# novara754/arctic-renderer

Measured on AMD Instinct MI355X. Metric: Mshaded-pixels/sec at 4K Sponza, 1 dir + 64 point lights; HBM GB/s vs roofline, higher is better.
Workload: dtype f32

## Files before the change

### arctic-renderer_amd/binding.py

```python
import ctypes as C
import os
import re

from .scene import CCreateInfo, CScene, CSettings

HERE = os.path.dirname(os.path.abspath(__file__))
LIB_PATH = os.environ.get("ARCTIC_HIP_LIBRARY") or os.path.join(HERE, "csrc", "libarctic_hip.so")
HEADER_PATH = os.path.join(os.path.dirname(HERE), "include", "arctic_hip.h")

OPTIONS = {"keep_float_output": 1, "count_light_evals": 2, "culling": 3, "debug": 4, "antialias": 5, "hdr16": 6, "ray_refit": 7, "shadow_cache": 9, "visbuffer": 10, "item_table_floor": 11, "light_path": 12, "markers": 13, "shadow_sharded": 14, "frames_in_flight": 15, "tiles_per_wave": 16, "tile_trace": 17, "raster_owner": 18, "tile_order": 19, "order_tail": 20, "sampler": 21, "texture_tiling": 22, "cluster_cull": 23, "small_triangles": 24, "env_lighting": 25, "point_shadow_size": 26, "texture_mips": 27}
TRACE_ANY, TRACE_BRUTE = 1, 2
ERRORS = {-1: "ARCTIC_E_INVALID", -2: "ARCTIC_E_DEVICE", -3: "ARCTIC_E_NO_DEVICE", -4: "ARCTIC_E_STATE", -5: "ARCTIC_E_CAPACITY"}

_vp, _u32, _u64, _i32, _i64 = C.c_void_p, C.c_uint32, C.c_uint64, C.c_int32, C.c_int64
_scene, _settings = C.POINTER(CScene), C.POINTER(CSettings)

SIGNATURES = {
    "arctic_create": (_vp, [C.POINTER(CCreateInfo), C.c_char_p, _u64]),
    "arctic_destroy": (None, [_vp]),
    "arctic_last_error": (C.c_char_p, [_vp]),
    "arctic_resize": (_i32, [_vp, _u32, _u32]),
    "arctic_flush": (_i32, [_vp]),
    "arctic_set_stream": (_i32, [_vp, _vp]),
    "arctic_use_own_stream": (_i32, [_vp]),
    "arctic_create_material": (_i32, [_vp, _vp, _u32, _u32, _vp, _u32, _u32, _vp, _u32, _u32]),
    "arctic_create_mesh": (_i32, [_vp, _vp, _u64, _vp, _u64, _u64]),
    "arctic_set_mesh_skin": (_i32, [_vp, _u64, _vp, _u64, _u32]),
    "arctic_set_mesh_pose": (_i32, [_vp, _u64, _vp, _u32]),
    "arctic_set_mesh_morph_targets": (_i32, [_vp, _u64, _vp, _u64, _u32]),
    "arctic_set_mesh_morph_weights": (_i32, [_vp, _u64, _vp, _u32]),
    "arctic_check_morph_targets": (_i32, [_vp, _u64, _u32]),
    "arctic_morph_vertices": (_i32, [_vp, _vp, _u64, _u32, _vp, _vp]),
    "arctic_read_mesh_vertices": (_i32, [_vp, _u64, _vp, _u64]),
    "arctic_check_mesh_skin": (_i32, [_vp, _u64, _u32]),
    "arctic_skin_vertices": (_i32, [_vp, _vp, _u64, _vp, _u32, _vp]),
    "arctic_set_material_extras": (_i32, [_vp, _u64, _vp, _vp, _u32, _u32, _vp, _u32, _u32]),
    "arctic_check_material_params": (_i32, [_vp]),
    "arctic_update_lights": (_i32, [_vp, _vp, _u64]),
    "arctic_update_spot_lights": (_i32, [_vp, _vp, _u64]),
    "arctic_spot_light_constants": (_i32, [_vp, _u64, _vp]),
    "arctic_update_point_shadow_lights": (_i32, [_vp, _vp, _u64]),
    "arctic_point_shadow_matrices": (_i32, [_vp, _vp]),
    "arctic_pass_point_shadows": (_i32, [_vp, _scene]),
    "arctic_read_point_shadow": (_i32, [_vp, _u32, _vp]),
    "arctic_write_point_shadow": (_i32, [_vp, _u32, _vp]),
    "arctic_create_hdri": (_i32, [_vp, _vp, _u32, _u32]),
    "arctic_render_frame": (_i32, [_vp, _scene, _settings, _vp]),
    "arctic_render_frame_device": (_i32, [_vp, _scene, _settings, _vp]),
    "arctic_pass_shadow_map": (_i32, [_vp, _scene]),
    "arctic_pass_gbuffer": (_i32, [_vp, _scene]),
    "arctic_pass_shade": (_i32, [_vp, _scene, _settings, _vp]),
    "arctic_post_process": (_i32, [_vp, _vp, _u32, _u32, _settings, _vp, _vp]),
    "arctic_antialias_device": (_i32, [_vp, _vp, _vp, _u32, _u32]),
# ... 76 lines not shown
```

### arctic-renderer_amd/csrc/common.h

```cpp
#pragma once
#include <hip/hip_runtime.h>
#include <stdint.h>
#include <stddef.h>
#include <algorithm>

namespace arctic {

constexpr int TILE = 8;
constexpr int TILE_PIXELS = 64;
constexpr uint32_t NO_MATERIAL = 0xFFFFFFFFu;
constexpr uint32_t MAX_TARGET = 16384;

struct GBuffer {
    float4 *a;
    float *b;
    float4 *c, *d, *e;
};
__host__ __device__ inline void gbuffer_pack(const float *v , uint32_t mat, float4 &A, float *B3, float4 &C, float4 &D, float4 &E) {
    A = make_float4(v[0], v[1], v[14], v[15]);
    B3[0] = v[16]; B3[1] = v[17]; B3[2] = __builtin_bit_cast(float, mat);
    C = make_float4(v[11], v[12], v[13], v[2]);
    D = make_float4(v[3], v[4], v[5], v[6]);
    E = make_float4(v[7], v[8], v[9], v[10]);
}
// ... 152 lines not shown
    const TexDesc *tex;
    const float2 *shadow_bounds;
    const float *shadow_map;
    uint8_t *out_rgba8;
    uint32_t shadow_size;
    uint32_t bounds_pitch;
    uint32_t width;
    uint32_t rows;
    uint32_t row0_in_tile;
    int32_t culling;
    int32_t hdr16;
    int32_t tm_method;
    float ambient;
    float inv_gamma;
    float exposure;
    uint32_t pad_c0;
    float *out_ldr;
    float *out_hdr;
    float eye[3];
    uint32_t n_lights;
    const float4 *light_pairs;
    const float4 *lights;
    float sun_dir[3];
    uint32_t n_spots;
    float sun_color[3];
    uint32_t n_cubes;
    const float *srgb_lut;
    union {
        unsigned long long *stats;
        const float4 *spots;
    };
// ... 7 lines not shown
    };
    uint32_t n_jobs;
    uint32_t cube_size;
    union {
        const unsigned long long *vis;
        const float *lod;
    };
    const SetupRec *recs; const RasterRec *rrecs; const uint32_t *rec_of; const ObjectRec *objs; const XVert *xv;
    const float4 *env;
    uint32_t env_w, env_h;
    float sky_fwd[3], sky_right[3], sky_up[3];
    float ndc_sx, ndc_sy;
    int32_t band_tiles, shard_index, shard_count, tile_y0;
    int32_t compact_tables;
};
static_assert(offsetof(ShadeParams, tex) == 64 && offsetof(ShadeParams, ambient) == 128 && offsetof(ShadeParams, sun_dir) == 192 &&
              offsetof(ShadeParams, srgb_lut) == 224, "ShadeParams: the blocks k_material loads in one batch each");
struct ShadeLaunch {
    hipStream_t stream;
    uint32_t loop;
    uint32_t from_vis;
    uint32_t stats;
    uint32_t tiles_per_wave;
    uint32_t env;
    uint32_t spot;
    uint32_t mip;
    uint32_t cube;
    uint32_t pbr;
};

// ... 21 lines not shown
    w = std::max(8u, std::min(W, 512u) >> (k - 1));
    h = std::max(4u, std::min(H, 256u) >> (k - 1));
}
inline uint32_t env_mip_count(uint32_t W, uint32_t H) { uint32_t n = 1; while (W > 1 || H > 1) { W = std::max(1u, W >> 1); H = std::max(1u, H >> 1); ++n; } return n; }
struct EnvBuild {
    const float4 *env; uint32_t W, H;
    float4 *levels;
    float2 *lut;
    float4 *mips;
    double *sh_rows;
    EnvTables *tables;
};
size_t env_levels_bytes(uint32_t W, uint32_t H);
size_t env_mips_bytes(uint32_t W, uint32_t H);
hipError_t launch_env_build(const EnvBuild &b, hipStream_t s);
constexpr uint32_t N_SHADE_STATS = 9;
constexpr uint32_t DEFAULT_TILES_PER_WAVE = 2;
constexpr uint32_t ORDER_NONE = 0xFFFFFFFFu;
__host__ __device__ inline uint32_t order_slot(uint32_t list, uint32_t i, uint32_t group) { return ((i / group) * 8u + list) * group + i % group; }
__host__ __device__ inline uint32_t order_slots(uint32_t tiles_x, uint32_t tiles_y, uint32_t group) {
    const uint32_t longest = ((tiles_x + 3) / 4) * ((tiles_y + 7) / 8);
    return 8u * ((longest + group - 1) / group * group);
}
constexpr uint32_t SMALL_FRAME_TILES = 48000;
inline uint32_t shadow_bounds_pitch(uint32_t S) { return S >= 4 && S <= 4900 ? (S + 3) / 4 : 0; }

hipError_t launch_vertex(const ObjectRec *objs, const uint32_t *block_obj, const uint32_t *block_first,
                         uint32_t n_blocks, const GeomParams &gp, XVert *xv, int clip_only, uint32_t *counters ,
                         unsigned long long *clear, unsigned long long clear_value, size_t clear_count ,
                         uint32_t *zero, size_t zero_count ,
                         const float *block_bounds , hipStream_t s);
// ... 57 lines not shown
```

### arctic-renderer_amd/csrc/renderer.cpp

```cpp
#include <algorithm>
#include <cstdarg>
#include <cstdio>
#include <dlfcn.h>

#include <cstdlib>
#include <cstring>
#include <cmath>
#include <limits>
#include <string>
#include <vector>

#include "../../include/arctic_hip.h"
#include "../../include/arctic_dist.h"
#include "common.h"
#include "ray_query.h"

using namespace arctic;

namespace {

struct Markers {
    int (*push)(const char *) = nullptr;
    int (*pop)() = nullptr;
    bool tried = false, on = false;
// ... 215 lines not shown
    uint32_t n_spots = 0;
    DevBuf d_cubes;
    uint32_t n_cubes = 0, cube_size = 1024;
    std::vector<ArcticPointShadowLight> cube_lights;
    std::vector<uint8_t> cube_key;
    uint32_t *h_cube_counts = nullptr, *dh_cube_counts = nullptr;
    uint32_t cube_count_faces = 0;
    DevBuf d_vis_set[3], d_p0, d_p1, d_p2, d_p3, d_p4, d_rgba8, d_ldr, d_hdr, d_counter;
    bool have_gbuffer = false, have_output = false, have_vis = false;
    int antialias = 0;
    DevBuf d_aa;
    bool output_filtered = false;
    bool aa_active() const { return antialias == 1 && rows() == height; }
    const void *rgba8_output() const { return output_filtered ? d_aa.p : d_rgba8.p; }
    int light_path = 0;
    bool visbuffer = true;
    PassTables tables[4];
    struct GeoSet {
        DevBuf d_xverts, d_recs, d_rrecs, d_clip_list, d_rec_of, d_items;
        DevBuf d_left;
        DevBuf d_bin_count, d_bin_slots;
        uint32_t item_cap = 0;
        uint32_t bins_x = 0, bins_y = 0;
        uint32_t n_tblocks = 0, n_vblocks = 0; bool cull_counted = false;
    } geo[4];
    DevBuf d_geo_counters, d_stage;
    hipStream_t shadow_stream = nullptr;
    hipEvent_t ev_fork = nullptr, ev_shadow = nullptr;
    hipEvent_t ev_skin = nullptr;
    uint64_t skin_seq = 0, skin_seen_shadow = 0, skin_seen_prepass[2] = {0, 0};
// ... 489 lines not shown
    std::memset(&sp, 0, sizeof sp);
    sp.g = r->gbuffer();
    const ArcticRenderer::GeoSet &G = r->geo[r->fwd()];
    sp.compact_tables = (G.d_recs.cap < (1ull << 32) && G.d_rrecs.cap < (1ull << 32) && G.d_xverts.cap < (1ull << 32) && G.d_rec_of.cap < (1ull << 32) &&
                         r->tables[r->fwd()].d.cap < (1ull << 32) && !(r->debug & 64)) ? 1 : 0;
    sp.vis = r->d_vis().as<unsigned long long>();
    if (!from_vis && r->mips_active()) sp.lod = r->d_lod.as<float>();
    sp.recs = G.d_recs.as<SetupRec>(); sp.rrecs = G.d_rrecs.as<RasterRec>(); sp.rec_of = G.d_rec_of.as<uint32_t>();
    sp.objs = r->tables[r->fwd()].objs; sp.xv = G.d_xverts.as<XVert>();
    sp.tex = r->d_tex.as<TexDesc>();
    sp.n_materials = (uint32_t)(r->tex.size() / 3);
    sp.srgb_lut = r->d_lut.as<float>();
    sp.shadow_map = r->shadow_size ? r->d_shadow().as<float>() : nullptr;
    sp.shadow_size = r->shadow_size;
    sp.lights = r->d_lights.as<float4>(); sp.light_pairs = r->d_light_pairs.as<float4>();
    sp.n_lights = r->n_lights;
    std::memcpy(sp.eye, sc->camera.eye, 12);
    dir_from_rot(sc->sun.rotation, sp.sun_dir);
    std::memcpy(sp.sun_color, sc->sun.color, 12);
    sp.ambient = sc->ambient;
    sp.tm_method = st->tm_method;
    sp.inv_gamma = 1.0f / st->gamma;
    sp.exposure = st->exposure;
    sp.width = r->width; sp.rows = r->rows(); sp.row0_in_tile = r->row0_in_tile;
    sp.tiles_x = r->tiles_x; sp.tiles_y = r->tiles_y;
    sp.out_rgba8 = static_cast<uint8_t *>(d_out && !r->aa_active() ? d_out : r->d_rgba8.p);
    size_t out_px = (size_t)r->rows() * r->width;
    if (r->keep_float) {
        HIPCHECK(r, r->d_ldr.ensure(out_px * 12));
        HIPCHECK(r, r->d_hdr.ensure(out_px * 12));
        sp.out_ldr = r->d_ldr.as<float>(); sp.out_hdr = r->d_hdr.as<float>();
// ... 60 lines not shown
        if (f.ptr && (f.ptr == static_cast<const void *>(sp.out_rgba8) || f.ptr == aa_out)) { HIPCHECK(r, hipStreamWaitEvent(r->stream, f.done, 0)); f.ptr = nullptr; }
    if (r->count_evals) {
        sp.stats = r->d_counter.as<unsigned long long>();
        HIPCHECK(r, hipMemsetAsync(r->d_counter.p, 0, 8 * N_SHADE_STATS, r->stream));
    }
    HIPCHECK(r, shade_once(r, sp, from_vis, r->count_evals != 0));
    if (aa) {
        Range aa_zone("Anti-aliasing Pass");
        HIPCHECK(r, launch_antialias(r->d_rgba8.p, aa_out, r->width, r->rows(), r->stream));
    }
    if (r->count_evals) {
        unsigned long long n[N_SHADE_STATS] = {};
        HIPCHECK(r, hipMemcpyAsync(n, r->d_counter.p, 8 * N_SHADE_STATS, hipMemcpyDeviceToHost, r->stream));
        HIPCHECK(r, hipStreamSynchronize(r->stream));
        r->stats[5] = n[0]; r->stats[6] = n[1]; r->stats[7] = n[2];
        r->light_stats[0] = n[3]; r->light_stats[1] = n[4];
        for (int i = 0; i < 4; ++i) r->edge_stats[i] = n[5 + i];
    }
    r->have_output = (d_out == nullptr);
    r->output_filtered = aa && d_out == nullptr;
    return ARCTIC_OK;
}

std::vector<uint8_t> shadow_inputs(const ArcticRenderer *r, const ArcticScene *sc) {
    std::vector<uint8_t> k;
    if (!r->shadow_size) return k;
    auto put = [&](const void *p, size_t n) { const uint8_t *b = static_cast<const uint8_t *>(p); k.insert(k.end(), b, b + n); };
    const uint64_t head[3] = {r->shadow_size, (uint64_t)r->meshes.size(), sc->n_objects};
    put(head, sizeof head);
    put(sc->sun.position, sizeof sc->sun.position);
    put(sc->sun.rotation, sizeof sc->sun.rotation);
// ... 556 lines not shown
    return ARCTIC_OK;
}

int arctic_read_mesh_vertices(ArcticRenderer *r, uint64_t mesh, ArcticVertex *out, uint64_t n_vertices) {
    if (!r) return ARCTIC_E_INVALID;
    if (mesh >= r->meshes.size()) return r->fail(ARCTIC_E_INVALID, "read_mesh_vertices: mesh %llu does not exist", (unsigned long long)mesh);
    const Mesh &m = r->meshes[mesh];
    if (!out || n_vertices != m.n_vertices) return r->fail(ARCTIC_E_INVALID, "read_mesh_vertices: room for %llu vertices, the mesh has %u", (unsigned long long)n_vertices, m.n_vertices);
    int rc = select_device(r);
    if (rc) return rc;
    HIPCHECK(r, hipStreamSynchronize(r->stream));
    HIPCHECK(r, hipMemcpy(out, m.vertices_in_use(), n_vertices * sizeof(ArcticVertex), hipMemcpyDeviceToHost));
    return ARCTIC_OK;
}

int arctic_update_lights(ArcticRenderer *r, const ArcticPointLight *lights, uint64_t n) {
    if (!r) return ARCTIC_E_INVALID;
    if (n && !lights) return r->fail(ARCTIC_E_INVALID, "update_lights: null");
    int rc = select_device(r);
    if (rc) return rc;
    uint32_t k = (uint32_t)std::min<uint64_t>(n, r->max_lights);
    HIPCHECK(r, hipStreamSynchronize(r->stream));
    if (k) HIPCHECK(r, hipMemcpy(r->d_lights.p, lights, (size_t)k * sizeof(ArcticPointLight), hipMemcpyHostToDevice));
    {
        const uint32_t n_pairs = (k + 1) / 2;
        std::vector<float> pairs((size_t)std::max(1u, n_pairs) * 12, 0.0f);
        for (uint32_t i = 0; i < 2 * n_pairs; ++i) {
            float *dst = pairs.data() + (size_t)(i / 2) * 12 + (i & 1);
            if (i < k) { dst[0] = lights[i].position[0]; dst[2] = lights[i].position[1]; dst[4] = lights[i].position[2];
                         dst[6] = lights[i].color[0]; dst[8] = lights[i].color[1]; dst[10] = lights[i].color[2]; }
            else { dst[0] = 0.0f; dst[2] = 1.0e6f; dst[4] = 0.0f; dst[6] = dst[8] = dst[10] = 0.0f; }
        }
        HIPCHECK(r, r->d_light_pairs.ensure(pairs.size() * 4));
        HIPCHECK(r, hipMemcpy(r->d_light_pairs.p, pairs.data(), pairs.size() * 4, hipMemcpyHostToDevice));
    }
    r->n_lights = k;
    return ARCTIC_OK;
}

int arctic_spot_light_constants(const ArcticSpotLight *lights, uint64_t n, float *out) {
    if (n && (!lights || !out)) return ARCTIC_E_INVALID;
    const float PI_F = (float)M_PI;
    for (uint64_t i = 0; i < n; ++i) {
        const ArcticSpotLight &l = lights[i];
        const float *f = l.position;
        for (int k = 0; k < 12; ++k) if (!std::isfinite(f[k])) return ARCTIC_E_INVALID;
        const double dx = l.direction[0], dy = l.direction[1], dz = l.direction[2];
        if (dx == 0.0 && dy == 0.0 && dz == 0.0) return ARCTIC_E_INVALID;
        if (!(l.inner_cone_angle >= 0.0f && l.inner_cone_angle <= l.outer_cone_angle && l.outer_cone_angle > 0.0f && l.outer_cone_angle <= PI_F &&
              l.range >= 0.0f)) return ARCTIC_E_INVALID;
// ... 636 lines not shown
            for (hipStream_t ps : r->prepass_stream) if (ps) HIPCHECK(r, hipStreamSynchronize(ps));
            if (r->own_stream_is_prepass()) HIPCHECK(r, hipStreamSynchronize(r->own_stream));
            if (r->cur >= (int)value) { r->cur = 0; r->have_vis = r->have_gbuffer = r->have_order = false; }
            r->released_valid[0] = r->released_valid[1] = r->released_valid[2] = false;
        }
        r->frames_in_flight = (int)value;
        break;
    case ARCTIC_OPT_MARKERS:
        g_markers.enable(value != 0);
        if (value && !g_markers.available()) return r->fail(ARCTIC_E_STATE, "set_option: libroctx64.so could not be loaded");
        break;
    case ARCTIC_OPT_LIGHT_PATH:
        if (value < 0 || value > 2) return r->fail(ARCTIC_E_INVALID, "set_option: light path must be 0..2");
        r->light_path = (int)value;
        break;
    case ARCTIC_OPT_ITEM_TABLE_FLOOR:
        if (value < 64 || value > 0x7FFFFFF0ll) return r->fail(ARCTIC_E_INVALID, "set_option: item table floor out of range");
        r->item_cap_floor = (uint32_t)value; r->geo[0].item_cap = r->geo[1].item_cap = r->geo[2].item_cap = r->geo[3].item_cap = 0;
        break;
    case ARCTIC_OPT_TILES_PER_WAVE:
        if (value < 0 || value > 64) return r->fail(ARCTIC_E_INVALID, "set_option: tiles per wave must be 0 (default) .. 64");
        r->tiles_per_wave = (uint32_t)value;
        break;
    case ARCTIC_OPT_TILE_TRACE: r->tile_trace = value != 0; break;
    case ARCTIC_OPT_TEXTURE_TILING: r->texture_tiling = value < 0 ? -1 : (value != 0); break;
    case ARCTIC_OPT_TEXTURE_MIPS:
        if (value < 0 || value > 1) return r->fail(ARCTIC_E_INVALID, "ARCTIC_OPT_TEXTURE_MIPS: 0 or 1");
        if ((int)value != r->texture_mips) r->lod_valid = false;
        r->texture_mips = (int)value;
        break;
// ... 531 lines not shown
```

### arctic-renderer_amd/csrc/shade.hip

```cpp
#include "common.h"
#include "edges.h"
#include "shadow_coords.h"
#include "texture_lod.h"

namespace arctic {

namespace {

typedef const ShadeParams __attribute__((address_space(4))) &SP;
typedef const ShadeParams __attribute__((address_space(4))) *KernArgs;

struct ArgsA { const float4 *ga; const float *gb; uint32_t tiles_x, tiles_y, T, stride; int32_t debug; uint32_t n_materials; };
__device__ __forceinline__ ArgsA args_a(KernArgs a) {
    ArgsA r = {a->g.a, a->g.b, a->tiles_x, a->tiles_y, a->tiles_per_wave, a->group_stride, a->debug, a->n_materials};
    asm volatile("" : "+s"(r.ga), "+s"(r.gb), "+s"(r.tiles_x), "+s"(r.tiles_y), "+s"(r.T), "+s"(r.stride), "+s"(r.debug), "+s"(r.n_materials));
    return r;
}
typedef const uint32_t __attribute__((address_space(4))) *OrderList;
struct OrderArgs { OrderList order; uint32_t n_jobs; };
__device__ __forceinline__ ArgsA args_a_first(KernArgs a, const float *&srgb_lut, const unsigned long long *&vis, OrderArgs &O) {
    ArgsA r = {a->g.a, a->g.b, a->tiles_x, a->tiles_y, a->tiles_per_wave, a->group_stride, a->debug, a->n_materials};
    srgb_lut = a->srgb_lut; vis = a->vis;
    const uint32_t *order = a->tile_order; O.n_jobs = a->n_jobs;
    asm volatile("" : "+s"(r.ga), "+s"(r.gb), "+s"(r.tiles_x), "+s"(r.tiles_y), "+s"(r.T), "+s"(r.stride), "+s"(r.debug), "+s"(r.n_materials), "+s"(srgb_lut), "+s"(vis),
// ... 22 lines not shown
struct ArgsC { float ambient; StoreArgs st; const float4 *gc, *gd, *ge; };
__device__ __forceinline__ ArgsC args_c(KernArgs a, const ArgsA &A, const ArgsB &B) {
    ArgsC r = {a->ambient, {B.hdr16, A.debug, B.tm, a->exposure, a->inv_gamma, a->out_ldr, a->out_hdr}, a->g.c, a->g.d, a->g.e};
    asm volatile("" : "+s"(r.ambient), "+s"(r.st.exposure), "+s"(r.st.inv_gamma), "+s"(r.st.out_ldr), "+s"(r.st.out_hdr), "+s"(r.gc), "+s"(r.gd), "+s"(r.ge));
    return r;
}
struct EpiArgs { StoreArgs st; uint8_t *out; uint32_t width, row0_in_tile; float ambient; };
__device__ __forceinline__ EpiArgs epi_args(KernArgs a) {
    EpiArgs r = {{a->hdr16, a->debug, a->tm_method, a->exposure, a->inv_gamma, a->out_ldr, a->out_hdr}, a->out_rgba8, a->width, a->row0_in_tile, a->ambient};
    asm volatile("" : "+s"(r.st.hdr16), "+s"(r.st.debug), "+s"(r.st.tm), "+s"(r.st.exposure), "+s"(r.st.inv_gamma), "+s"(r.st.out_ldr), "+s"(r.st.out_hdr), "+s"(r.out),
                 "+s"(r.width), "+s"(r.row0_in_tile), "+s"(r.ambient));
    return r;
}
__device__ __forceinline__ ShadowArgs shadow_args(SP sp) { ShadowArgs r = {sp.shadow_map, sp.shadow_bounds, sp.shadow_size, sp.bounds_pitch}; return r; }
__device__ __forceinline__ StoreArgs store_args(SP sp) { StoreArgs r = {sp.hdr16, sp.debug, sp.tm_method, sp.exposure, sp.inv_gamma, sp.out_ldr, sp.out_hdr}; return r; }
struct LightArgs { float eye[3]; uint32_t n_lights; const float4 *pairs, *lights; };
__device__ __forceinline__ LightArgs light_args(SP sp) {
    LightArgs r = {{sp.eye[0], sp.eye[1], sp.eye[2]}, sp.n_lights, sp.light_pairs, sp.lights};
    asm volatile("" : "+s"(r.eye[0]), "+s"(r.eye[1]), "+s"(r.eye[2]), "+s"(r.n_lights), "+s"(r.pairs), "+s"(r.lights));
    return r;
}
struct SunArgs { float dir[3], color[3]; };
__device__ __forceinline__ SunArgs sun_args(SP sp) {
    SunArgs r = {{sp.sun_dir[0], sp.sun_dir[1], sp.sun_dir[2]}, {sp.sun_color[0], sp.sun_color[1], sp.sun_color[2]}};
    asm volatile("" : "+s"(r.dir[0]), "+s"(r.dir[1]), "+s"(r.dir[2]), "+s"(r.color[0]), "+s"(r.color[1]), "+s"(r.color[2]));
    return r;
}

struct f3 { float x, y, z; };
__device__ __forceinline__ f3 mk(float x, float y, float z) { f3 r; r.x = x; r.y = y; r.z = z; return r; }
__device__ __forceinline__ f3 operator+(f3 a, f3 b) { return mk(a.x + b.x, a.y + b.y, a.z + b.z); }
__device__ __forceinline__ f3 operator-(f3 a, f3 b) { return mk(a.x - b.x, a.y - b.y, a.z - b.z); }
__device__ __forceinline__ f3 operator*(f3 a, f3 b) { return mk(a.x * b.x, a.y * b.y, a.z * b.z); }
__device__ __forceinline__ f3 operator*(f3 a, float s) { return mk(a.x * s, a.y * s, a.z * s); }
// ... 365 lines not shown
    k.q21 = (v2){p.q2, p.q1}; k.q0_ = (v2){p.q0, 0.0f};
    return k;
}
typedef float f4v __attribute__((ext_vector_type(4)));
__device__ __forceinline__ void load_light_pair(const char *p , f4v &A, f4v &B, f4v &C) {
    asm volatile("s_load_dwordx4 %0, %3, 0x0\n\ts_load_dwordx4 %1, %3, 0x10\n\ts_load_dwordx4 %2, %3, 0x20" : "=&s"(A), "=&s"(B), "=&s"(C) : "s"(p));
}
__device__ __forceinline__ void wait_and_sub(v2 lx, v2 ly, v2 lz, v2 w_xy, v2 wz, v2 &dx, v2 &dy, v2 &dz) {
    asm volatile("s_waitcnt lgkmcnt(0)\n\t"
                 "v_pk_add_f32 %0, %3, %6 op_sel:[0,0] op_sel_hi:[1,0] neg_lo:[0,1] neg_hi:[0,1]\n\t"
                 "v_pk_add_f32 %1, %4, %6 op_sel:[0,1] op_sel_hi:[1,1] neg_lo:[0,1] neg_hi:[0,1]\n\t"
                 "v_pk_add_f32 %2, %5, %7 op_sel:[0,0] op_sel_hi:[1,0] neg_lo:[0,1] neg_hi:[0,1]"
                 : "=&v"(dx), "=&v"(dy), "=&v"(dz) : "s"(lx), "s"(ly), "s"(lz), "v"(w_xy), "v"(wz));
}

__device__ __forceinline__ v2 accumulate_pair(const PackedPix &k, v2 dx, v2 dy, v2 dz, v2 cr, v2 cg, v2 cb, Sums2 &S) {
    const v2 d2 = pk_fma(dz, dz, pk_fma(dy, dy, dx * dx));
    v2 ndx;
    const v2 inv = rsq2_and_mul_b0(d2, dx, k.n_xy, ndx);
    const v2 nd = pk_fma_b1<0>(dz, k.nz_wox, pk_fma_b1<1>(dy, k.n_xy, ndx));
    const v2 ndwi = pk_mul_sat(nd, inv);
    const v2 hx = pk_fma_b2<1>(dx, inv, k.nz_wox), hy = pk_fma_b2<0>(dy, inv, k.wo_yz), hz = pk_fma_b2<1>(dz, inv, k.wo_yz);
    const v2 hh = pk_fma(hz, hz, pk_fma(hy, hy, hx * hx));
    v2 q;
    const v2 rh = rsq2_and_fma_b01(hh, ndwi, k.q21, q);
    const v2 m = pk_fma(hh * rh, (v2){-0.5f, -0.5f}, (v2){1.0f, 1.0f});
    const v2 ex = pk_fnma_b2<0>(hx, rh, k.n_xy), ey = pk_fnma_b2<1>(hy, rh, k.n_xy), ez = pk_fnma_b2<0>(hz, rh, k.nz_wox);
    const v2 e2 = pk_fma(ez, ez, pk_fma(ey, ey, ex * ex));
    const v2 dd = pk_fma_b2<1>(e2, pk_fma_b12<1, 0>(e2, k.oma2_c4, k.oma2_c4), k.wz_a2);
    const v2 den = (dd * dd) * pk_fma_b2<0>(q, ndwi, k.q0_);
    const v2 sc = ndwi * (inv * inv);
    v2 m2;
    const v2 rden = rcp2_and_mul(den, m, m, m2);
    const v2 p5 = m2 * m2 * m;
    const v2 s2 = (sc * ndwi) * rden;
    const v2 s1 = pk_fma(-sc, p5, sc), s3 = s2 * p5;
    pk_fma_s(cr, s1, S.a[0]); pk_fma_s(cg, s1, S.a[1]); pk_fma_s(cb, s1, S.a[2]);
    pk_fma_s(cr, s2, S.b[0]); pk_fma_s(cg, s2, S.b[1]); pk_fma_s(cb, s2, S.b[2]);
    pk_fma_s(cr, s3, S.c[0]); pk_fma_s(cg, s3, S.c[1]); pk_fma_s(cb, s3, S.c[2]);
    return nd;
}

__device__ __forceinline__ float rrt_odt(float c) {
    float a = fm(c, c + 0.0245786f, -0.000090537f);
    float b = fm(c, fm(0.983729f, c, 0.4329510f), 0.238081f);
    return a * rcp(b);
}
__device__ __forceinline__ v2 pk_fma_sat(v2 k , v2 a, v2 c) { v2 r; asm("v_pk_fma_f32 %0, %1, %2, %3 clamp" : "=v"(r) : "s"(k), "v"(a), "v"(c)); return r; }
__device__ __forceinline__ float fma_sat(float k , float a, float c) { float r; asm("v_fma_f32 %0, %1, %2, %3 clamp" : "=v"(r) : "s"(k), "v"(a), "v"(c)); return r; }
__device__ __forceinline__ f3 tonemap(f3 c, int tm, float exposure) {
    f3 t;
    if (tm == 1) {
        const float LOG2E = 1.4426950408889634f;
        const f3 x = mk(c.x * exposure, c.y * exposure, c.z * exposure);
// ... 178 lines not shown
        C[0] = __builtin_fmaf(cr, s3, C[0]); C[1] = __builtin_fmaf(cg, s3, C[1]); C[2] = __builtin_fmaf(cb, s3, C[2]);
    }
}
template <int LOOP, bool STATS, bool SPOT = false, bool CUBE = false, bool PBR = false>
__device__ __forceinline__ f3 lit_radiance(SP sp, uint32_t lane, float nr, float ng, float nb, float rough, float metal, f3 base,
                                           const float4 &gc, const float4 &gd, const float4 &ge, float nscale = 1.0f ) {
    const f3 n = PBR ? get_normal_scaled(nr, ng, nb, gc, gd, ge, nscale) : get_normal(nr, ng, nb, gc, gd, ge);
    const f3 world = mk(gc.x, gc.y, gc.z);
    const LightArgs la = light_args(sp);
    const f3 wo = normalize(mk(la.eye[0], la.eye[1], la.eye[2]) - world);
    asm volatile("" : "+v"(metal));
    LoopPix px;
    TailPix tp;
    make_pix(n, wo, world, base, metal, rough, px, tp);
    unsigned long long contributing = 0ull, wave_zero = 0ull;
    f3 Lo;
    if (LOOP == 1) {
        Sums S;
        {
            const SunArgs sun = sun_args(sp);
            const f3 d = mk(-sun.dir[0], -sun.dir[1], -sun.dir[2]);
            float s1, s2, s3;
            light_scalars<false>(px, d, dot(n, d), s1, s2, s3);
            for (int k = 0; k < 3; ++k) { S.a[k] = sun.color[k] * s1; S.b[k] = sun.color[k] * s2; S.c[k] = sun.color[k] * s3; }
        }
        for (uint32_t i = 0; i < la.n_lights; ++i) {
            typedef const f4v __attribute__((address_space(4))) *const_f4;
            const f4v lp = ((const_f4)la.lights)[2 * i], lc = ((const_f4)la.lights)[2 * i + 1];
            const f3 dl = mk(lp.x, lp.y, lp.z) - world;
            const float ndl = dot(n, dl);
// ... 2 lines not shown
            float s1, s2, s3;
            light_scalars<true>(px, dl, ndl, s1, s2, s3);
            S.a[0] = __builtin_fmaf(lc.x, s1, S.a[0]); S.a[1] = __builtin_fmaf(lc.y, s1, S.a[1]); S.a[2] = __builtin_fmaf(lc.z, s1, S.a[2]);
            S.b[0] = __builtin_fmaf(lc.x, s2, S.b[0]); S.b[1] = __builtin_fmaf(lc.y, s2, S.b[1]); S.b[2] = __builtin_fmaf(lc.z, s2, S.b[2]);
            S.c[0] = __builtin_fmaf(lc.x, s3, S.c[0]); S.c[1] = __builtin_fmaf(lc.y, s3, S.c[1]); S.c[2] = __builtin_fmaf(lc.z, s3, S.c[2]);
        }
        if (SPOT) spot_sums(sp, px, S.a, S.b, S.c);
        if (CUBE) cube_sums(sp, px, S.a, S.b, S.c);
        Lo = resolve_sums(tp, S.a, S.b, S.c);
    } else {
        Sums2 S;
        for (int k = 0; k < 3; ++k) { S.a[k] = (v2){0.0f, 0.0f}; S.b[k] = (v2){0.0f, 0.0f}; S.c[k] = (v2){0.0f, 0.0f}; }
        const uint32_t n_pairs = (la.n_lights + 1) >> 1;
        const PackedPix pk = pack_pix(px);
        const char *lp = reinterpret_cast<const char *>(la.pairs);
        auto finish = [&](v2 dx, v2 dy, v2 dz, const f4v &Bq, const f4v &C, uint32_t p) {
            const v2 nd = accumulate_pair(pk, dx, dy, dz, (v2){Bq.z, Bq.w}, (v2){C.x, C.y}, (v2){C.z, C.w}, S);
            if (STATS) {
                const bool second = 2 * p + 1 < la.n_lights;
                const unsigned long long m0 = __ballot(nd.x > 0.0f), m1 = second ? __ballot(nd.y > 0.0f) : ~0ull;
                contributing += __popcll(m0) + (second ? __popcll(m1) : 0);
                wave_zero += (m0 == 0ull ? 1 : 0) + (m1 == 0ull ? 1 : 0);
            }
        };
        if (n_pairs) {
            f4v A0, B0, C0, A1, B1, C1;
            v2 dx, dy, dz;
            load_light_pair(lp, A0, B0, C0);
            for (uint32_t p = 0;;) {
                wait_and_sub((v2){A0.x, A0.y}, (v2){A0.z, A0.w}, (v2){B0.x, B0.y}, pk.w_xy, pk.wz_a2, dx, dy, dz);
                if (p + 1 < n_pairs) load_light_pair(lp + 48 * (p + 1), A1, B1, C1);
                finish(dx, dy, dz, B0, C0, p);
                if (++p == n_pairs) break;
                wait_and_sub((v2){A1.x, A1.y}, (v2){A1.z, A1.w}, (v2){B1.x, B1.y}, pk.w_xy, pk.wz_a2, dx, dy, dz);
                if (p + 1 < n_pairs) load_light_pair(lp + 48 * (p + 1), A0, B0, C0);
                finish(dx, dy, dz, B1, C1, p);
                if (++p == n_pairs) break;
            }
            asm volatile("s_waitcnt lgkmcnt(0)");
        }
        float A[3], Bs[3], Cs[3];
        {
            const SunArgs sun = sun_args(sp);
            const f3 d = mk(-sun.dir[0], -sun.dir[1], -sun.dir[2]);
            float s1, s2, s3;
            light_scalars<false>(px, d, dot(n, d), s1, s2, s3);
            for (int k = 0; k < 3; ++k) {
                A[k] = __builtin_fmaf(sun.color[k], s1, S.a[k].x + S.a[k].y);
                Bs[k] = __builtin_fmaf(sun.color[k], s2, S.b[k].x + S.b[k].y);
                Cs[k] = __builtin_fmaf(sun.color[k], s3, S.c[k].x + S.c[k].y);
            }
        }
        if (SPOT) spot_sums(sp, px, A, Bs, Cs);
        if (CUBE) cube_sums(sp, px, A, Bs, Cs);
        Lo = resolve_sums(tp, A, Bs, Cs);
    }
    if (STATS) {
        const unsigned long long active = __ballot(1);
        if (lane == (uint32_t)__ffsll((long long)active) - 1) {
            atomicAdd(sp.stats, (unsigned long long)__popcll(active) * la.n_lights);
            atomicAdd(sp.stats + 1, (unsigned long long)__popcll(active));
            atomicAdd(sp.stats + 2, contributing);
            atomicAdd(sp.stats + 3, wave_zero);
            atomicAdd(sp.stats + 4, 1ull);
        }
    }
    return Lo;
}

__device__ __forceinline__ f3 env_level(const EnvTables *T, uint32_t k, float u, float v) {
    const float4 *img = T->level[k];
    const uint32_t w = T->w[k], h = T->h[k];
    int x0, x1, y0, y1;
    float fx, fy;
    wrap_axis(u, w, x0, x1, fx);
    wrap_axis(v, h, y0, y1, fy);
    const float4 a = img[(size_t)y0 * w + x0], b = img[(size_t)y0 * w + x1], c = img[(size_t)y1 * w + x0], d = img[(size_t)y1 * w + x1];
    const float gx = 1.0f - fx, gy = 1.0f - fy;
    const float w00 = gx * gy, w10 = fx * gy, w01 = gx * fy, w11 = fx * fy;
// ... 731 lines not shown
```

### include/arctic_hip.h

```cpp
#ifndef ARCTIC_HIP_H
#define ARCTIC_HIP_H

#include <stdint.h>

#ifdef __cplusplus
extern "C" {
#endif

#define ARCTIC_OK            0
#define ARCTIC_E_INVALID    -1
#define ARCTIC_E_DEVICE     -2
#define ARCTIC_E_NO_DEVICE  -3
#define ARCTIC_E_STATE      -4
#define ARCTIC_E_CAPACITY   -5


typedef struct ArcticCamera {
    float eye[3];
    float rotation[2];
    float aspect;
    float fov_y;
    float z_near_far[2];
} ArcticCamera;

// ... 131 lines not shown
    float base_color_factor[3];
    float metallic_factor;
    float roughness_factor;
    float normal_scale;
    float occlusion_strength;
    float emissive_factor[3];
    float reserved[2];
} ArcticMaterialParams;
int arctic_set_material_extras(ArcticRenderer *r, uint64_t material, const ArcticMaterialParams *params,
                               const void *emissive_rgba8, uint32_t ew, uint32_t eh,
                               const void *occlusion_rgba8, uint32_t ow, uint32_t oh);

int arctic_check_material_params(const ArcticMaterialParams *params);

int arctic_update_lights(ArcticRenderer *r, const ArcticPointLight *lights, uint64_t n);

int arctic_update_spot_lights(ArcticRenderer *r, const ArcticSpotLight *lights, uint64_t n);

int arctic_spot_light_constants(const ArcticSpotLight *lights, uint64_t n, float *out);

int arctic_update_point_shadow_lights(ArcticRenderer *r, const ArcticPointShadowLight *lights, uint64_t n);

int arctic_point_shadow_matrices(const ArcticPointShadowLight *light, float *out96);

int arctic_create_hdri(ArcticRenderer *r, const float *rgba32f, uint32_t w, uint32_t h);


int arctic_render_frame(ArcticRenderer *r, const ArcticScene *scene,
                        const ArcticSettings *settings, uint8_t *out_rgba8);

// ... 26 lines not shown

int arctic_read_point_shadow(ArcticRenderer *r, uint32_t light, float *faces);
int arctic_write_point_shadow(ArcticRenderer *r, uint32_t light, const float *faces);

int arctic_read_output(ArcticRenderer *r, float *ldr_rgb, float *hdr_rgb, uint8_t *rgba8);

int arctic_frame_constants(const ArcticScene *scene, float *proj_view, float *light_proj_view, float *sun_dir);

int arctic_stats(ArcticRenderer *r, uint64_t *out, uint32_t n);

#define ARCTIC_OPT_KEEP_FLOAT_OUTPUT 1
#define ARCTIC_OPT_COUNT_LIGHT_EVALS 2
#define ARCTIC_OPT_CULLING           3
#define ARCTIC_OPT_DEBUG             4
#define ARCTIC_OPT_HDR16             6
#define ARCTIC_OPT_SHADOW_CACHE      9
#define ARCTIC_OPT_FRAMES_IN_FLIGHT  15
#define ARCTIC_OPT_VISBUFFER        10
#define ARCTIC_OPT_ITEM_TABLE_FLOOR 11
#define ARCTIC_OPT_LIGHT_PATH       12
#define ARCTIC_OPT_TILES_PER_WAVE    16
#define ARCTIC_OPT_TILE_TRACE        17
#define ARCTIC_OPT_RASTER_OWNER      18
#define ARCTIC_OPT_TILE_ORDER        19
#define ARCTIC_OPT_ORDER_TAIL        20
#define ARCTIC_OPT_SAMPLER           21
#define ARCTIC_OPT_TEXTURE_TILING    22
#define ARCTIC_OPT_CLUSTER_CULL      23
#define ARCTIC_OPT_SMALL_TRIANGLES   24
#define ARCTIC_OPT_MARKERS          13
// ... 71 lines not shown
```

Baseline: 44640.

## Group point-light pairs by zero color channel and skip dead channel FMAs

On the host, point lights are sorted into pairs grouped by which RGB channel is zero for both lights in a pair. The run boundaries are packed into a shade parameter. The packed light loop is split into four runs, each templated to skip the accumulation FMAs for the channel known to be zero. This reduces per-pixel arithmetic when light colors have zero channels, at the cost of more code paths and larger kernel code.

```diff
diff --git a/arctic-renderer_amd/binding.py b/arctic-renderer_amd/binding.py
--- a/arctic-renderer_amd/binding.py
+++ b/arctic-renderer_amd/binding.py
@@ -8,7 +8,7 @@
 LIB_PATH = os.environ.get("ARCTIC_HIP_LIBRARY") or os.path.join(HERE, "csrc", "libarctic_hip.so")
 HEADER_PATH = os.path.join(os.path.dirname(HERE), "include", "arctic_hip.h")
 
-OPTIONS = {"keep_float_output": 1, "count_light_evals": 2, "culling": 3, "debug": 4, "antialias": 5, "hdr16": 6, "ray_refit": 7, "shadow_cache": 9, "visbuffer": 10, "item_table_floor": 11, "light_path": 12, "markers": 13, "shadow_sharded": 14, "frames_in_flight": 15, "tiles_per_wave": 16, "tile_trace": 17, "raster_owner": 18, "tile_order": 19, "order_tail": 20, "sampler": 21, "texture_tiling": 22, "cluster_cull": 23, "small_triangles": 24, "env_lighting": 25, "point_shadow_size": 26, "texture_mips": 27}
+OPTIONS = {"keep_float_output": 1, "count_light_evals": 2, "culling": 3, "debug": 4, "antialias": 5, "hdr16": 6, "ray_refit": 7, "light_pair_runs": 8, "shadow_cache": 9, "visbuffer": 10, "item_table_floor": 11, "light_path": 12, "markers": 13, "shadow_sharded": 14, "frames_in_flight": 15, "tiles_per_wave": 16, "tile_trace": 17, "raster_owner": 18, "tile_order": 19, "order_tail": 20, "sampler": 21, "texture_tiling": 22, "cluster_cull": 23, "small_triangles": 24, "env_lighting": 25, "point_shadow_size": 26, "texture_mips": 27}
 TRACE_ANY, TRACE_BRUTE = 1, 2
 ERRORS = {-1: "ARCTIC_E_INVALID", -2: "ARCTIC_E_DEVICE", -3: "ARCTIC_E_NO_DEVICE", -4: "ARCTIC_E_STATE", -5: "ARCTIC_E_CAPACITY"}
 
@@ -37,6 +37,7 @@
     "arctic_set_material_extras": (_i32, [_vp, _u64, _vp, _vp, _u32, _u32, _vp, _u32, _u32]),
     "arctic_check_material_params": (_i32, [_vp]),
     "arctic_update_lights": (_i32, [_vp, _vp, _u64]),
+    "arctic_light_pair_table": (_i32, [_vp, _u64, _i32, _vp, _vp, _vp]),
     "arctic_update_spot_lights": (_i32, [_vp, _vp, _u64]),
     "arctic_spot_light_constants": (_i32, [_vp, _u64, _vp]),
     "arctic_update_point_shadow_lights": (_i32, [_vp, _vp, _u64]),
diff --git a/arctic-renderer_amd/csrc/common.h b/arctic-renderer_amd/csrc/common.h
--- a/arctic-renderer_amd/csrc/common.h
+++ b/arctic-renderer_amd/csrc/common.h
@@ -190,7 +190,7 @@
     float ambient;
     float inv_gamma;
     float exposure;
-    uint32_t pad_c0;
+    uint32_t pair_runs;
     float *out_ldr;
     float *out_hdr;
     float eye[3];
@@ -228,6 +228,7 @@
     int32_t band_tiles, shard_index, shard_count, tile_y0;
     int32_t compact_tables;
 };
+constexpr uint32_t PAIR_RUN_BITS = 10, PAIR_RUN_MAX = (1u << PAIR_RUN_BITS) - 1;
 static_assert(offsetof(ShadeParams, tex) == 64 && offsetof(ShadeParams, ambient) == 128 && offsetof(ShadeParams, sun_dir) == 192 &&
               offsetof(ShadeParams, srgb_lut) == 224, "ShadeParams: the blocks k_material loads in one batch each");
 struct ShadeLaunch {
@@ -279,7 +280,7 @@
 size_t env_levels_bytes(uint32_t W, uint32_t H);
 size_t env_mips_bytes(uint32_t W, uint32_t H);
 hipError_t launch_env_build(const EnvBuild &b, hipStream_t s);
-constexpr uint32_t N_SHADE_STATS = 9;
+constexpr uint32_t N_SHADE_STATS = 10;
 constexpr uint32_t DEFAULT_TILES_PER_WAVE = 2;
 constexpr uint32_t ORDER_NONE = 0xFFFFFFFFu;
 __host__ __device__ inline uint32_t order_slot(uint32_t list, uint32_t i, uint32_t group) { return ((i / group) * 8u + list) * group + i % group; }
diff --git a/arctic-renderer_amd/csrc/renderer.cpp b/arctic-renderer_amd/csrc/renderer.cpp
--- a/arctic-renderer_amd/csrc/renderer.cpp
+++ b/arctic-renderer_amd/csrc/renderer.cpp
@@ -253,6 +253,9 @@
     bool aa_active() const { return antialias == 1 && rows() == height; }
     const void *rgba8_output() const { return output_filtered ? d_aa.p : d_rgba8.p; }
     int light_path = 0;
+    int light_pair_runs = 1;
+    std::vector<ArcticPointLight> h_lights;
+    uint32_t pair_runs = 0;
     bool visbuffer = true;
     PassTables tables[4];
     struct GeoSet {
@@ -772,7 +775,7 @@
     sp.shadow_map = r->shadow_size ? r->d_shadow().as<float>() : nullptr;
     sp.shadow_size = r->shadow_size;
     sp.lights = r->d_lights.as<float4>(); sp.light_pairs = r->d_light_pairs.as<float4>();
-    sp.n_lights = r->n_lights;
+    sp.n_lights = r->n_lights; sp.pair_runs = r->pair_runs;
     std::memcpy(sp.eye, sc->camera.eye, 12);
     dir_from_rot(sc->sun.rotation, sp.sun_dir);
     std::memcpy(sp.sun_color, sc->sun.color, 12);
@@ -863,7 +866,7 @@
         HIPCHECK(r, hipMemcpyAsync(n, r->d_counter.p, 8 * N_SHADE_STATS, hipMemcpyDeviceToHost, r->stream));
         HIPCHECK(r, hipStreamSynchronize(r->stream));
         r->stats[5] = n[0]; r->stats[6] = n[1]; r->stats[7] = n[2];
-        r->light_stats[0] = n[3]; r->light_stats[1] = n[4];
+        r->light_stats[0] = n[3]; r->light_stats[1] = n[4]; r->stats[4] = n[9];
         for (int i = 0; i < 4; ++i) r->edge_stats[i] = n[5 + i];
     }
     r->have_output = (d_out == nullptr);
@@ -1450,6 +1453,71 @@
     return ARCTIC_OK;
 }
 
+namespace {
+constexpr uint32_t PAIR_PARTNER = 0xFFFFFFFFu;
+uint32_t zero_channels(const ArcticPointLight &l) {
+    uint32_t m = 0;
+    for (int c = 0; c < 3; ++c) { uint32_t b; std::memcpy(&b, &l.color[c], 4); m |= (b == 0u ? 1u : 0u) << c; }
+    return m;
+}
+uint32_t run_of_mask(uint32_t m) { return m & 1u ? 0u : m & 2u ? 1u : m & 4u ? 2u : 3u; }
+void light_pair_table(const ArcticPointLight *lights, uint32_t k, bool runs, std::vector<uint32_t> &slots, std::vector<uint32_t> &masks, uint32_t run_end[3]) {
+    const uint32_t n_pairs = (k + 1) / 2;
+    std::vector<uint32_t> seq; seq.reserve(2 * (size_t)n_pairs);
+    if (runs && n_pairs <= PAIR_RUN_MAX) {
+        for (uint32_t c = 0; c < 4; ++c)
+            for (uint32_t i = 0; i < k; ++i) if (run_of_mask(zero_channels(lights[i])) == c) seq.push_back(i);
+    } else {
+        runs = false;
+        for (uint32_t i = 0; i < k; ++i) seq.push_back(i);
+    }
+    if (k & 1u) seq.push_back(PAIR_PARTNER);
+    auto mask_of = [&](uint32_t s) { return s == PAIR_PARTNER ? 7u : zero_channels(lights[s]); };
+    slots.clear(); masks.clear();
+    uint32_t end[4] = {0, 0, 0, 0};
+    for (uint32_t c = 0; c < 4; ++c) {
+        for (uint32_t p = 0; p < n_pairs; ++p) {
+            const uint32_t a = seq[2 * p], b = seq[2 * p + 1], m = mask_of(a) & mask_of(b);
+            if ((runs && b != PAIR_PARTNER ? run_of_mask(m) : 3u) != c) continue;
+            slots.push_back(a); slots.push_back(b); masks.push_back(m);
+        }
+        end[c] = (uint32_t)masks.size();
+    }
+    run_end[0] = end[0]; run_end[1] = end[1]; run_end[2] = end[2];
+}
+}
+
+int arctic_light_pair_table(const ArcticPointLight *lights, uint64_t n, int32_t runs, uint32_t *slots, uint32_t *masks, uint32_t *run_end) {
+    if ((n && !lights) || n > 0x7FFFFFFFull || (n && (!slots || !masks)) || !run_end) return ARCTIC_E_INVALID;
+    std::vector<uint32_t> s, m;
+    light_pair_table(lights, (uint32_t)n, runs != 0, s, m, run_end);
+    if (!s.empty()) std::memcpy(slots, s.data(), s.size() * 4);
+    if (!m.empty()) std::memcpy(masks, m.data(), m.size() * 4);
+    return ARCTIC_OK;
+}
+
+namespace {
+int upload_light_pairs(ArcticRenderer *r) {
+    const ArcticPointLight *lights = r->h_lights.data();
+    const uint32_t k = (uint32_t)r->h_lights.size(), n_pairs = (k + 1) / 2;
+    std::vector<uint32_t> slots, masks;
+    uint32_t run_end[3];
+    light_pair_table(lights, k, r->light_pair_runs != 0, slots, masks, run_end);
+    std::vector<float> pairs((size_t)std::max(1u, n_pairs) * 12, 0.0f);
+    for (uint32_t i = 0; i < 2 * n_pairs; ++i) {
+        float *dst = pairs.data() + (size_t)(i / 2) * 12 + (i & 1);
+        const uint32_t s = slots[i];
+        if (s != PAIR_PARTNER) { dst[0] = lights[s].position[0]; dst[2] = lights[s].position[1]; dst[4] = lights[s].position[2];
+                                 dst[6] = lights[s].color[0]; dst[8] = lights[s].color[1]; dst[10] = lights[s].color[2]; }
+        else { dst[0] = 0.0f; dst[2] = 1.0e6f; dst[4] = 0.0f; dst[6] = dst[8] = dst[10] = 0.0f; }
+    }
+    HIPCHECK(r, r->d_light_pairs.ensure(pairs.size() * 4));
+    HIPCHECK(r, hipMemcpy(r->d_light_pairs.p, pairs.data(), pairs.size() * 4, hipMemcpyHostToDevice));
+    r->pair_runs = run_end[0] | run_end[1] << PAIR_RUN_BITS | run_end[2] << (2 * PAIR_RUN_BITS);
+    return ARCTIC_OK;
+}
+}
+
 int arctic_update_lights(ArcticRenderer *r, const ArcticPointLight *lights, uint64_t n) {
     if (!r) return ARCTIC_E_INVALID;
     if (n && !lights) return r->fail(ARCTIC_E_INVALID, "update_lights: null");
@@ -1458,18 +1526,8 @@
     uint32_t k = (uint32_t)std::min<uint64_t>(n, r->max_lights);
     HIPCHECK(r, hipStreamSynchronize(r->stream));
     if (k) HIPCHECK(r, hipMemcpy(r->d_lights.p, lights, (size_t)k * sizeof(ArcticPointLight), hipMemcpyHostToDevice));
-    {
-        const uint32_t n_pairs = (k + 1) / 2;
-        std::vector<float> pairs((size_t)std::max(1u, n_pairs) * 12, 0.0f);
-        for (uint32_t i = 0; i < 2 * n_pairs; ++i) {
-            float *dst = pairs.data() + (size_t)(i / 2) * 12 + (i & 1);
-            if (i < k) { dst[0] = lights[i].position[0]; dst[2] = lights[i].position[1]; dst[4] = lights[i].position[2];
-                         dst[6] = lights[i].color[0]; dst[8] = lights[i].color[1]; dst[10] = lights[i].color[2]; }
-            else { dst[0] = 0.0f; dst[2] = 1.0e6f; dst[4] = 0.0f; dst[6] = dst[8] = dst[10] = 0.0f; }
-        }
-        HIPCHECK(r, r->d_light_pairs.ensure(pairs.size() * 4));
-        HIPCHECK(r, hipMemcpy(r->d_light_pairs.p, pairs.data(), pairs.size() * 4, hipMemcpyHostToDevice));
-    }
+    r->h_lights.assign(lights, lights + k);
+    if ((rc = upload_light_pairs(r)) != ARCTIC_OK) return rc;
     r->n_lights = k;
     return ARCTIC_OK;
 }
@@ -2136,6 +2194,16 @@
         if (value < 0 || value > 2) return r->fail(ARCTIC_E_INVALID, "set_option: light path must be 0..2");
         r->light_path = (int)value;
         break;
+    case ARCTIC_OPT_LIGHT_PAIR_RUNS: {
+        if (value < 0 || value > 1) return r->fail(ARCTIC_E_INVALID, "ARCTIC_OPT_LIGHT_PAIR_RUNS: 0 or 1");
+        if ((int)value == r->light_pair_runs) break;
+        int rc = select_device(r);
+        if (rc) return rc;
+        HIPCHECK(r, hipStreamSynchronize(r->stream));
+        r->light_pair_runs = (int)value;
+        if ((rc = upload_light_pairs(r)) != ARCTIC_OK) return rc;
+        break;
+    }
     case ARCTIC_OPT_ITEM_TABLE_FLOOR:
         if (value < 64 || value > 0x7FFFFFF0ll) return r->fail(ARCTIC_E_INVALID, "set_option: item table floor out of range");
         r->item_cap_floor = (uint32_t)value; r->geo[0].item_cap = r->geo[1].item_cap = r->geo[2].item_cap = r->geo[3].item_cap = 0;
diff --git a/arctic-renderer_amd/csrc/shade.hip b/arctic-renderer_amd/csrc/shade.hip
--- a/arctic-renderer_amd/csrc/shade.hip
+++ b/arctic-renderer_amd/csrc/shade.hip
@@ -1,3 +1,4 @@
+#include <type_traits>
 #include "common.h"
 #include "edges.h"
 #include "shadow_coords.h"
@@ -60,10 +61,10 @@
 }
 __device__ __forceinline__ ShadowArgs shadow_args(SP sp) { ShadowArgs r = {sp.shadow_map, sp.shadow_bounds, sp.shadow_size, sp.bounds_pitch}; return r; }
 __device__ __forceinline__ StoreArgs store_args(SP sp) { StoreArgs r = {sp.hdr16, sp.debug, sp.tm_method, sp.exposure, sp.inv_gamma, sp.out_ldr, sp.out_hdr}; return r; }
-struct LightArgs { float eye[3]; uint32_t n_lights; const float4 *pairs, *lights; };
+struct LightArgs { float eye[3]; uint32_t n_lights; const float4 *pairs, *lights; uint32_t pair_runs; };
 __device__ __forceinline__ LightArgs light_args(SP sp) {
-    LightArgs r = {{sp.eye[0], sp.eye[1], sp.eye[2]}, sp.n_lights, sp.light_pairs, sp.lights};
-    asm volatile("" : "+s"(r.eye[0]), "+s"(r.eye[1]), "+s"(r.eye[2]), "+s"(r.n_lights), "+s"(r.pairs), "+s"(r.lights));
+    LightArgs r = {{sp.eye[0], sp.eye[1], sp.eye[2]}, sp.n_lights, sp.light_pairs, sp.lights, sp.pair_runs};
+    asm volatile("" : "+s"(r.eye[0]), "+s"(r.eye[1]), "+s"(r.eye[2]), "+s"(r.n_lights), "+s"(r.pairs), "+s"(r.lights), "+s"(r.pair_runs));
     return r;
 }
 struct SunArgs { float dir[3], color[3]; };
@@ -459,6 +460,7 @@
                  : "=&v"(dx), "=&v"(dy), "=&v"(dz) : "s"(lx), "s"(ly), "s"(lz), "v"(w_xy), "v"(wz));
 }
 
+template <int SKIP>
 __device__ __forceinline__ v2 accumulate_pair(const PackedPix &k, v2 dx, v2 dy, v2 dz, v2 cr, v2 cg, v2 cb, Sums2 &S) {
     const v2 d2 = pk_fma(dz, dz, pk_fma(dy, dy, dx * dx));
     v2 ndx;
@@ -480,9 +482,9 @@
     const v2 p5 = m2 * m2 * m;
     const v2 s2 = (sc * ndwi) * rden;
     const v2 s1 = pk_fma(-sc, p5, sc), s3 = s2 * p5;
-    pk_fma_s(cr, s1, S.a[0]); pk_fma_s(cg, s1, S.a[1]); pk_fma_s(cb, s1, S.a[2]);
-    pk_fma_s(cr, s2, S.b[0]); pk_fma_s(cg, s2, S.b[1]); pk_fma_s(cb, s2, S.b[2]);
-    pk_fma_s(cr, s3, S.c[0]); pk_fma_s(cg, s3, S.c[1]); pk_fma_s(cb, s3, S.c[2]);
+    if (SKIP != 0) pk_fma_s(cr, s1, S.a[0]); if (SKIP != 1) pk_fma_s(cg, s1, S.a[1]); if (SKIP != 2) pk_fma_s(cb, s1, S.a[2]);
+    if (SKIP != 0) pk_fma_s(cr, s2, S.b[0]); if (SKIP != 1) pk_fma_s(cg, s2, S.b[1]); if (SKIP != 2) pk_fma_s(cb, s2, S.b[2]);
+    if (SKIP != 0) pk_fma_s(cr, s3, S.c[0]); if (SKIP != 1) pk_fma_s(cg, s3, S.c[1]); if (SKIP != 2) pk_fma_s(cb, s3, S.c[2]);
     return nd;
 }
 
@@ -691,6 +693,7 @@
     TailPix tp;
     make_pix(n, wo, world, base, metal, rough, px, tp);
     unsigned long long contributing = 0ull, wave_zero = 0ull;
+    uint32_t skip_trips = 0;
     f3 Lo;
     if (LOOP == 1) {
         Sums S;
@@ -723,8 +726,8 @@
         const uint32_t n_pairs = (la.n_lights + 1) >> 1;
         const PackedPix pk = pack_pix(px);
         const char *lp = reinterpret_cast<const char *>(la.pairs);
-        auto finish = [&](v2 dx, v2 dy, v2 dz, const f4v &Bq, const f4v &C, uint32_t p) {
-            const v2 nd = accumulate_pair(pk, dx, dy, dz, (v2){Bq.z, Bq.w}, (v2){C.x, C.y}, (v2){C.z, C.w}, S);
+        auto finish = [&](auto skip, v2 dx, v2 dy, v2 dz, const f4v &Bq, const f4v &C, uint32_t p) {
+            const v2 nd = accumulate_pair<decltype(skip)::value>(pk, dx, dy, dz, (v2){Bq.z, Bq.w}, (v2){C.x, C.y}, (v2){C.z, C.w}, S);
             if (STATS) {
                 const bool second = 2 * p + 1 < la.n_lights;
                 const unsigned long long m0 = __ballot(nd.x > 0.0f), m1 = second ? __ballot(nd.y > 0.0f) : ~0ull;
@@ -733,19 +736,32 @@
             }
         };
         if (n_pairs) {
+            const uint32_t run_mask = (1u << PAIR_RUN_BITS) - 1;
+            const uint32_t end_r = min(la.pair_runs & run_mask, n_pairs), end_g = min((la.pair_runs >> PAIR_RUN_BITS) & run_mask, n_pairs),
+                           end_b = min((la.pair_runs >> (2 * PAIR_RUN_BITS)) & run_mask, n_pairs);
+            if (STATS) skip_trips = end_b;
             f4v A0, B0, C0, A1, B1, C1;
-            v2 dx, dy, dz;
+            uint32_t p = 0;
             load_light_pair(lp, A0, B0, C0);
-            for (uint32_t p = 0;;) {
-                wait_and_sub((v2){A0.x, A0.y}, (v2){A0.z, A0.w}, (v2){B0.x, B0.y}, pk.w_xy, pk.wz_a2, dx, dy, dz);
-                if (p + 1 < n_pairs) load_light_pair(lp + 48 * (p + 1), A1, B1, C1);
-                finish(dx, dy, dz, B0, C0, p);
-                if (++p == n_pairs) break;
-                wait_and_sub((v2){A1.x, A1.y}, (v2){A1.z, A1.w}, (v2){B1.x, B1.y}, pk.w_xy, pk.wz_a2, dx, dy, dz);
-                if (p + 1 < n_pairs) load_light_pair(lp + 48 * (p + 1), A0, B0, C0);
-                finish(dx, dy, dz, B1, C1, p);
-                if (++p == n_pairs) break;
-            }
+            auto trip = [&](auto skip, const f4v &A, const f4v &B, const f4v &C, f4v &An, f4v &Bn, f4v &Cn) {
+                v2 dx, dy, dz;
+                wait_and_sub((v2){A.x, A.y}, (v2){A.z, A.w}, (v2){B.x, B.y}, pk.w_xy, pk.wz_a2, dx, dy, dz);
+                if (p + 1 < n_pairs) load_light_pair(lp + 48 * (p + 1), An, Bn, Cn);
+                finish(skip, dx, dy, dz, B, C, p);
+                ++p;
+            };
+            auto run = [&](auto skip, uint32_t end) {
+                if (p < end && (p & 1u)) trip(skip, A1, B1, C1, A0, B0, C0);
+                while (p < end) {
+                    trip(skip, A0, B0, C0, A1, B1, C1);
+                    if (p == end) break;
+                    trip(skip, A1, B1, C1, A0, B0, C0);
+                }
+            };
+            run(std::integral_constant<int, 0>{}, end_r);
+            run(std::integral_constant<int, 1>{}, end_g);
+            run(std::integral_constant<int, 2>{}, end_b);
+            run(std::integral_constant<int, 3>{}, n_pairs);
             asm volatile("s_waitcnt lgkmcnt(0)");
         }
         float A[3], Bs[3], Cs[3];
@@ -772,6 +788,7 @@
             atomicAdd(sp.stats + 2, contributing);
             atomicAdd(sp.stats + 3, wave_zero);
             atomicAdd(sp.stats + 4, 1ull);
+            if (LOOP == 2) atomicAdd(sp.stats + 9, (unsigned long long)skip_trips);
         }
     }
     return Lo;
diff --git a/include/arctic_hip.h b/include/arctic_hip.h
--- a/include/arctic_hip.h
+++ b/include/arctic_hip.h
@@ -169,6 +169,7 @@
 int arctic_check_material_params(const ArcticMaterialParams *params);
 
 int arctic_update_lights(ArcticRenderer *r, const ArcticPointLight *lights, uint64_t n);
+int arctic_light_pair_table(const ArcticPointLight *lights, uint64_t n, int32_t runs, uint32_t *slots, uint32_t *masks, uint32_t *run_end);
 
 int arctic_update_spot_lights(ArcticRenderer *r, const ArcticSpotLight *lights, uint64_t n);
 
@@ -225,6 +226,7 @@
 #define ARCTIC_OPT_CULLING           3
 #define ARCTIC_OPT_DEBUG             4
 #define ARCTIC_OPT_HDR16             6
+#define ARCTIC_OPT_LIGHT_PAIR_RUNS   8
 #define ARCTIC_OPT_SHADOW_CACHE      9
 #define ARCTIC_OPT_FRAMES_IN_FLIGHT  15
 #define ARCTIC_OPT_VISBUFFER        10
```

Result: faster. 45680 (median of 6 runs) (+2.3%).
